# NUStatBioinfo/DegNorm

Hardware: AMD Instinct MI355X
Metric: genes/sec (20k genes x 10 samples, 5 iters) (higher is better)
Workload: dtype f64

## Files before the change

degnorm_amd/_lib.py:

```python
import ctypes
import os
import numpy as np

_HERE = os.path.dirname(os.path.abspath(__file__))
LIB_PATH = os.environ.get('DN_LIB_PATH') or os.path.join(_HERE, 'libdegnorm_amd.so')
TRACE_LEN = 48

DN_OK = 0
DN_E_INVALID, DN_E_HIP, DN_E_STATE, DN_E_UNSUPPORTED, DN_E_NO_DEVICE = -1, -2, -3, -4, -5

NMF_RANK_ONE, NMF, NMF_RATIO = 0, 1, 2
STATUS_NAMES = {0: 'ok', -1: 'ArpackError (all-zero matrix)', -2: 'empty minimum (no |K| >= 1e-5)',
                -3: 'ValueError (fewer than 2 rows or columns)', -4: 'ArpackNoConvergence (solver step cap)'}

EXIT_NAMES = ('low_cov', 'zero_sample', 'median', 'no_loop', 'refined', 'refine_fallback', 'not_found_fallback')

_lib = None


class DegnormAmdError(RuntimeError):
    pass


class Params(ctypes.Structure):
# ... 46 lines not shown
    lib.dn_debug_peek.argtypes = [vp, i32, vp]
    lib.dn_last_kernel_ms.argtypes = [vp]
    lib.dn_last_kernel_ms.restype = dbl
    lib.dn_main_kernel_name.argtypes = [vp]
    lib.dn_main_kernel_name.restype = c.c_char_p
    lib.dn_last_span_ms.argtypes = [vp]
    lib.dn_last_span_ms.restype = dbl
    lib.dn_last_init_ms.argtypes = [vp]
    lib.dn_last_init_ms.restype = dbl
    lib.dn_init_kernel_name.argtypes = [vp]
    lib.dn_init_kernel_name.restype = c.c_char_p
    lib.dn_split_length.argtypes = [vp]
    lib.dn_split_length.restype = i32
    lib.dn_class_lengths.argtypes = [vp, i32, i32, P(i32), P(i32)]
    lib.dn_class_tier_cols.argtypes = [vp, c.c_int, P(i32), P(i32)]
    lib.dn_tiny_length.argtypes = [vp]
    lib.dn_tiny_length.restype = i32
    lib.dn_class_kernel_ms.argtypes = [vp, c.c_int]
    lib.dn_class_kernel_ms.restype = dbl
    lib.dn_class_kernel_name.argtypes = [vp, c.c_int]
    lib.dn_class_kernel_name.restype = c.c_char_p
    lib.dn_synchronize.argtypes = [vp]
    lib.dn_measure_copy_gbps.argtypes = [vp, i64, c.c_int]
    lib.dn_measure_copy_gbps.restype = dbl
    lib.dn_last_rowmax_ms.argtypes = [vp]
    lib.dn_last_rowmax_ms.restype = dbl
    lib.dn_measure_read_gbps.argtypes = [vp, i64, c.c_int]
    lib.dn_measure_read_gbps.restype = dbl
    lib.dn_assemble_coverage.argtypes = [c.c_int, i64, i32, P(i64), P(vp), P(vp), i64, P(i64), i64, P(i32), P(i64), P(i64), P(i32),
                                         P(c.c_float), P(dbl)]
# ... 445 lines not shown
        return int(self.lib.dn_split_length(self.h))

    def class_lengths(self, p, downsample_rate=1):
        a, b = ctypes.c_int32(0), ctypes.c_int32(0)
        _check(self.lib.dn_class_lengths(self.h, int(p), int(downsample_rate), ctypes.byref(a), ctypes.byref(b)))
        return int(a.value), int(b.value)

    def class_tier_cols(self, cls):
        a, b = ctypes.c_int32(0), ctypes.c_int32(0)
        _check(self.lib.dn_class_tier_cols(self.h, int(cls), ctypes.byref(a), ctypes.byref(b)))
        return int(a.value), int(b.value)

    def tiny_length(self):
        return int(self.lib.dn_tiny_length(self.h))

    def class_kernel_ms(self, cls):
        return float(self.lib.dn_class_kernel_ms(self.h, int(cls)))

    def class_kernel_name(self, cls):
        return self.lib.dn_class_kernel_name(self.h, int(cls)).decode()

    def measure_copy_gbps(self, nbytes=1 << 30, reps=5):
        return float(self.lib.dn_measure_copy_gbps(self.h, int(nbytes), int(reps)))

    def measure_read_gbps(self, nbytes=1 << 30, reps=5):
        return float(self.lib.dn_measure_read_gbps(self.h, int(nbytes), int(reps)))

    def last_rowmax_ms(self):
        return float(self.lib.dn_last_rowmax_ms(self.h))
```

degnorm_amd/csrc/dn_api.hip:

```cpp
#include "dn_kernels.hpp"
#include "dn_host.hpp"
#include "../../include/degnorm_amd.h"

#include <dlfcn.h>
#include <rccl/rccl.h>

#include <algorithm>
#include <atomic>
#include <cmath>
#include <cstdio>
#include <cstdlib>
#include <cstring>
#include <memory>
#include <numeric>
#include <string>
#include <thread>
#include <vector>

#ifndef DN_P_MAX_TEMPLATED
#define DN_P_MAX_TEMPLATED 64
#endif
#define DN_P_2_16(X)  X(2) X(3) X(4) X(5) X(6) X(7) X(8) X(9) X(10) X(11) X(12) X(13) X(14) X(15) X(16)
#define DN_P_17_24(X) X(17) X(18) X(19) X(20) X(21) X(22) X(23) X(24)
#define DN_P_25_32(X) X(25) X(26) X(27) X(28) X(29) X(30) X(31) X(32)
// ... 419 lines not shown

static thread_local std::string g_err;

int dn::fail(int code, const std::string &msg) { g_err = msg; return code; }
int dn::fail_hip(const char *what, hipError_t e) { return fail(DN_E_HIP, std::string(what) + ": " + hipGetErrorString(e)); }
void dn::clear_error() { g_err.clear(); }
const char *dn::last_error() { return g_err.c_str(); }
using dn::fail;

struct dn_handle_s {
    int device = -1;
    int n_cus = 0;
    static constexpr int NCLS = 3;
    dn::Stream stream[NCLS];
    dn::Event ev_start[NCLS], ev_end[NCLS];
    dn::Event ev_ready, ev_i0, ev_i1;
    const dn::KernelSet *ks = nullptr;

    int64_t n = 0;
    int32_t p = 0;
    int64_t total = 0;
    int32_t lmax = 0;
    std::vector<int64_t> goff;
    std::vector<int32_t> glen;
    std::vector<int64_t> svoff;

    struct GeneClass {
        const dn::KernelSet *ks = nullptr;
        int32_t n = 0;
        int32_t longest = 0;
        dn::DeviceBuffer<int32_t> d_order;
        std::vector<int32_t> order;
        dn::DeviceBuffer<int32_t> d_counter;
        dn::DeviceBuffer<char> d_ws;
        int slots = 0;
        int32_t S = 0;
        int64_t slot_bytes = 0;
        int32_t lds_cols = 0;
        size_t dyn_lds = 0;
        float last_ms = 0.f;
    };
    struct DataSet {
        dn::DeviceBuffer<float> d_cov;
        dn::DeviceBuffer<int64_t> d_goff;
        dn::DeviceBuffer<int32_t> d_glen;
        dn::DeviceBuffer<int32_t> d_order;
        dn::DeviceBuffer<int32_t> d_counter;
        dn::DeviceBuffer<int64_t> d_ds;
        dn::DeviceBuffer<double> d_rho;
        dn::DeviceBuffer<int32_t> d_flags;
        dn::DeviceBuffer<int32_t> d_trace;
        dn::DeviceBuffer<double> d_kfin;
        dn::DeviceBuffer<int32_t> d_emode;
        dn::DeviceBuffer<double> d_svec;
        dn::DeviceBuffer<int64_t> d_svoff;
        dn::DeviceBuffer<float> d_rowmax;
        dn::DeviceBuffer<int32_t> d_x16;
        dn::DeviceBuffer<double> d_rhoc, d_xw, d_xadj, d_part, d_pvec;
        dn::DeviceBuffer<double> d_scales;
        dn::DeviceBuffer<double> d_x;
        dn::DeviceBuffer<uint8_t> d_ran;
        int32_t n_iter = 0;
        dn::DeviceBuffer<double> d_est_sums, d_cov_sums;
        dn::DeviceBuffer<int32_t> d_status;
        dn::DeviceBuffer<double> d_est;
        dn::DeviceBuffer<int32_t> d_tile_gene, d_tile_col;
        GeneClass cls[NCLS];
        bool have_estimate_state = false;
        dn::PinnedBuffer<int32_t> host_trace;
        size_t host_trace_len = 0;
        dn::DeviceBuffer<int32_t> d_trace_head;
// ... 163 lines not shown
    return n;
}

int dn_p_supported(int p) { return p <= dn::P_MAX && dn::kernel_set_for(p) != nullptr; }
int dn_p_max(void) { return dn::P_WIDE_MAX; }

static int create_streams(dn_handle h)
{
    int prio_least = 0, prio_greatest = 0;
    DN_TRY(hipDeviceGetStreamPriorityRange(&prio_least, &prio_greatest));
    const int prio[dn_handle_s::NCLS] = {prio_greatest, (prio_least + prio_greatest) / 2, prio_least};
    for (int c = 0; c < dn_handle_s::NCLS; c++) {
        DN_TRY(h->stream[c].create(hipStreamCreateWithPriority, hipStreamNonBlocking, prio[c]));
        DN_TRY(h->ev_start[c].create(hipEventCreate));
        DN_TRY(h->ev_end[c].create(hipEventCreate));
    }
    DN_TRY(h->ev_ready.create(hipEventCreateWithFlags, hipEventDisableTiming));
    DN_TRY(h->ev_i0.create(hipEventCreate));
    DN_TRY(h->ev_i1.create(hipEventCreate));
    return DN_OK;
}

int dn_create(int device, dn_handle *out)
{
    if (!out) return fail(DN_E_INVALID, "dn_create: out is null");
    *out = nullptr;
    int ndev = 0;
    if (hipGetDeviceCount(&ndev) != hipSuccess || ndev <= 0) return fail(DN_E_NO_DEVICE, "no HIP device visible");
    if (device < 0 || device >= ndev) return fail(DN_E_INVALID, "dn_create: device index out of range");
    DN_TRY(hipSetDevice(device));
// ... 210 lines not shown
        for (int32_t g : order) {
            const int32_t L = h->glen[g];
            ord[(h->split_len > 0 && L <= h->split_len) ? ((pair && L <= h->tiny_len) ? 2 : 1) : 0].push_back(g);
        }
        h->data.cls[0].ks = h->ks;
        h->data.cls[1].ks = (h->ks->p != 0 && h->split_len > 0) ? dn::kernel_set_narrow(p) : nullptr;
        h->data.cls[2].ks = pair;
        if (ord[0].size() >= 8) {
            const size_t n0 = ord[0].size();
            std::vector<int32_t> mixed;
            mixed.reserve(n0);
            for (size_t i = 0, j = n0 - 1; i < j; i++, j--) { mixed.push_back(ord[0][i]); mixed.push_back(ord[0][j]); }
            if (n0 & 1) mixed.push_back(ord[0][n0 / 2]);
            ord[0] = mixed;
        }
        for (int c = 0; c < dn_handle_s::NCLS; c++) {
            auto &C = h->data.cls[c];
            C.n = (int32_t) ord[c].size();
            if (C.n == 0 || !C.ks) { C.n = 0; continue; }
            DN_TRY(C.d_order.alloc(sizeof(int32_t) * (size_t) C.n));
            DN_TRY(C.d_counter.alloc(sizeof(int32_t) * 4));
            DN_TRY(hipMemcpy(C.d_order, ord[c].data(), sizeof(int32_t) * (size_t) C.n, hipMemcpyHostToDevice));
            C.order = ord[c];
            int32_t cols = C.longest = h->glen[ord[c][0]];
            if (C.ks == dn::kernel_set_rows()) cols = (cols + h->ds_hint - 1) / h->ds_hint;
            const int rc = size_class(h, C, cols);
            if (rc != DN_OK) return rc;
        }
        if (h->data.cls[0].n == 0 && (h->data.cls[1].n > 0 || h->data.cls[2].n > 0) && h->ks->p == 0) return fail(DN_E_STATE, "internal: empty wide class for the generic kernels");
        return DN_OK;
    });
    if (rc != DN_OK) {
        const std::string msg = g_err;
        free_device(h);
        h->n = 0; h->total = 0;
        return fail(rc, msg);
    }
    return DN_OK;
}

static int check_shape(dn_handle h, int64_t n_genes, int32_t p, const int64_t *lengths)
{
// ... 112 lines not shown
}

int dn_baseline_iteration(dn_handle h, const double *scale, const dn_params *prm, const int64_t *ds_start,
                          double *rho, int32_t *flags, int32_t *trace)
{
    if (!h || !h->data.d_cov) return fail(DN_E_STATE, "dn_baseline_iteration: nothing uploaded");
    if (!scale || !prm) return fail(DN_E_INVALID, "dn_baseline_iteration: null argument");
    if ((rho == nullptr) != (flags == nullptr)) return fail(DN_E_INVALID, "dn_baseline_iteration: rho and flags are fetched together or not at all");
    { const int rc = check_params(prm, ds_start, h->n, [&](int64_t g) { return h->glen[g]; }); if (rc != DN_OK) return rc; }
    for (int i = 0; i < h->p; i++) if (!(scale[i] > 0.0) || !std::isfinite(scale[i])) return fail(DN_E_INVALID, "scale factors must be positive and finite");
    DN_TRY(hipSetDevice(h->device));
    return synced_classes(h, [&]() -> int {
        const int32_t rate = prm->downsample_rate;
        for (auto &C : h->data.cls) {
            if (C.n == 0 || !C.ks) continue;
            const int32_t longest = C.longest;
            const int32_t need = rate > 1 ? (longest + rate - 1) / rate : longest;
            if (need > C.S) {
                DN_TRY(hipStreamSynchronize(h->stream[0]));
                const int rc = size_class(h, C, need);
                if (rc != DN_OK) return rc;
            }
        }
        if (prm->want_estimates && !h->data.d_svec)
            DN_TRY(h->data.d_svec.alloc(sizeof(double) * (size_t) std::max<int64_t>(h->svoff[h->n], 1)));

        dn::IterArgs a;
        std::memset(&a, 0, sizeof(a));
        a.cov = h->data.d_cov; a.goff = h->data.d_goff; a.glen = h->data.d_glen; a.order = h->data.d_order; a.counter = h->data.d_counter;
        a.ds_start = nullptr;
        a.ws = h->data.cls[0].d_ws; a.rho = h->data.d_rho; a.flags = h->data.d_flags; a.trace = h->data.d_trace; a.kfin = h->data.d_kfin; a.emode = h->data.d_emode;
// ... 19 lines not shown
            const double per_call = 4.0 * (double) (C.ks->nt > 0 ? C.ks->nt : 128);
            std::vector<std::pair<double, int32_t>> key((size_t) C.n);
            for (int32_t k = 0; k < C.n; k++) {
                const int32_t g = C.order[k];
                const int32_t *tr = &h->data.host_trace[(size_t) g * h->trace_cols];
                key[k] = {(double) tr[2] + per_call * (double) tr[1] + 1e-3 * (double) h->glen[g], g};
            }
            std::stable_sort(key.begin(), key.end(), [](const std::pair<double, int32_t> &a, const std::pair<double, int32_t> &b) { return a.first > b.first; });
            for (int32_t k = 0; k < C.n; k++) C.order[k] = key[k].second;
            DN_TRY(hipMemcpyAsync(C.d_order, C.order.data(), sizeof(int32_t) * (size_t) C.n, hipMemcpyHostToDevice, h->stream[0]));
        }
        DN_TRY(hipMemsetAsync(h->data.d_trace, 0, sizeof(int32_t) * (size_t) h->n * dn::TRACE_LEN, h->stream[0]));
        for (auto &C : h->data.cls) if (C.n > 0) DN_TRY(hipMemsetAsync(C.d_counter, 0, sizeof(int32_t) * 4, h->stream[0]));
        DN_TRY(hipEventRecord(h->ev_ready, h->stream[0]));
        int first_cls = -1;
        for (int c = 0; c < dn_handle_s::NCLS; c++) {
            auto &C = h->data.cls[c];
            C.last_ms = 0.f;
            if (C.n == 0) continue;
            if (first_cls < 0) first_cls = c;
            hipStream_t st = h->stream[c];
            if (c > 0) DN_TRY(hipStreamWaitEvent(st, h->ev_ready, 0));
            a.order = C.d_order; a.counter = C.d_counter; a.ws = C.d_ws; a.slot_bytes = C.slot_bytes; a.S = C.S;
            a.lds_cols = C.lds_cols; a.n_genes = C.n;
            DN_TRY(hipEventRecord(h->ev_start[c], st));
            const int lrc = C.ks->baseline_ptr ? C.ks->baseline_ptr(a, h->data.d_scales, C.slots, st) : C.ks->baseline(a, C.slots, C.dyn_lds, st);
            if (lrc != 0) return fail(DN_E_HIP, std::string("k_baseline launch: ") + hipGetErrorString((hipError_t) lrc));
            DN_TRY(hipEventRecord(h->ev_end[c], st));
        }
        for (int c = 1; c < dn_handle_s::NCLS; c++)
            if (h->data.cls[c].n > 0) DN_TRY(hipStreamWaitEvent(h->stream[0], h->ev_end[c], 0));
        if (rho) {
            DN_TRY(hipMemcpyAsync(rho, h->data.d_rho, sizeof(double) * (size_t) h->n * h->p, hipMemcpyDeviceToHost, h->stream[0]));
            DN_TRY(hipMemcpyAsync(flags, h->data.d_flags, sizeof(int32_t) * (size_t) h->n, hipMemcpyDeviceToHost, h->stream[0]));
        }
        const int32_t tcols = h->trace_cols;
        const size_t trace_ints = (size_t) h->n * (size_t) tcols;
        if (h->data.host_trace_len < trace_ints) {
            h->data.host_trace_len = 0;
            DN_TRY(h->data.host_trace.alloc(sizeof(int32_t) * trace_ints));
            h->data.host_trace_len = trace_ints;
        }
        if (tcols == dn::TRACE_LEN)
            DN_TRY(hipMemcpyAsync(h->data.host_trace, h->data.d_trace, sizeof(int32_t) * trace_ints, hipMemcpyDeviceToHost, h->stream[0]));
        else {
            if (!h->data.d_trace_head) DN_TRY(h->data.d_trace_head.alloc(sizeof(int32_t) * (size_t) h->n * dn::TRACE_LEN));
            hipLaunchKernelGGL(k_trace_head, dim3((unsigned) std::min<size_t>(1024, (trace_ints + 255) / 256)), dim3(256), 0, h->stream[0],
                               h->data.d_trace, h->data.d_trace_head, (long long) trace_ints, (int) tcols);
            DN_TRY(hipGetLastError());
            DN_TRY(hipMemcpyAsync(h->data.host_trace, h->data.d_trace_head, sizeof(int32_t) * trace_ints, hipMemcpyDeviceToHost, h->stream[0]));
        }
        DN_TRY(hipStreamSynchronize(h->stream[0]));
        h->have_trace = (prm->downsample_rate <= 1);
        if (trace) std::memcpy(trace, h->data.host_trace, sizeof(int32_t) * trace_ints);
        h->last_span_ms = 0.f;
        for (int c = 0; c < dn_handle_s::NCLS; c++) {
            if (h->data.cls[c].n == 0) continue;
            DN_TRY(hipEventElapsedTime(&h->data.cls[c].last_ms, h->ev_start[c], h->ev_end[c]));
            float span = 0.f;
            DN_TRY(hipEventElapsedTime(&span, h->ev_start[first_cls], h->ev_end[c]));
            h->last_span_ms = std::max(h->last_span_ms, span);
        }
        h->last_ms = first_cls >= 0 ? h->data.cls[first_cls].last_ms : 0.f;
        h->data.have_estimate_state = prm->want_estimates != 0;
        return DN_OK;
    });
}
// ... 565 lines not shown
        return DN_OK;
    });
}

double dn_last_f64_ms(dn_handle h) { return h ? (double) h->last_f64_ms : 0.0; }

double dn_last_kernel_ms(dn_handle h) { return h ? (double) h->last_ms : 0.0; }
double dn_last_init_ms(dn_handle h) { return h ? (double) h->last_init_ms : 0.0; }
double dn_last_span_ms(dn_handle h) { return h ? (double) h->last_span_ms : 0.0; }
double dn_last_rowmax_ms(dn_handle h) { return h ? (double) h->last_rowmax_ms : 0.0; }
const char *dn_init_kernel_name(dn_handle h) { return h ? h->init_name : ""; }
const char *dn_main_kernel_name(dn_handle h) { return (h && h->ks) ? h->ks->baseline_name : ""; }
double dn_class_kernel_ms(dn_handle h, int cls) { return (h && cls >= 0 && cls < dn_handle_s::NCLS) ? (double) h->data.cls[cls].last_ms : 0.0; }
const char *dn_class_kernel_name(dn_handle h, int cls) { return (h && cls >= 0 && cls < dn_handle_s::NCLS && h->data.cls[cls].ks && h->data.cls[cls].n > 0) ? h->data.cls[cls].ks->baseline_name : ""; }
int32_t dn_tiny_length(dn_handle h) { return h ? h->tiny_len : 0; }
int dn_class_tier_cols(dn_handle h, int cls, int32_t *reg_cols, int32_t *lds_cols)
{
    if (!h || cls < 0 || cls >= dn_handle_s::NCLS || !reg_cols || !lds_cols) return fail(DN_E_INVALID, "dn_class_tier_cols: bad argument");
    const auto &C = h->data.cls[cls];
    const bool live = C.ks && C.n > 0;
    *reg_cols = live ? C.ks->reg_tier_cols : 0;
    *lds_cols = live ? C.lds_cols : 0;
    return DN_OK;
}
int dn_class_lengths(dn_handle h, int32_t p, int32_t downsample_rate, int32_t *split_len, int32_t *tiny_len)
{
    if (!h || !split_len || !tiny_len) return fail(DN_E_INVALID, "dn_class_lengths: null argument");
    const dn::KernelSet *ks = dn::kernel_set_for(p);
    if (!ks) return fail(DN_E_UNSUPPORTED, "no kernels compiled for p = " + std::to_string(p));
    DN_TRY(hipSetDevice(h->device));
// ... 104 lines not shown
```

degnorm_amd/csrc/dn_kernels.hpp:

```cpp
#pragma once
#include <hip/hip_runtime.h>
#include <stddef.h>
#include <stdint.h>
#include <type_traits>
#include "dn_reduce.hpp"
#include "dn_dpp_ops.hpp"

#ifdef DN_MARKS
#define DN_MARK(name) asm volatile("; DN_MARK " name)
#else
#define DN_MARK(name)
#endif

namespace dn {

constexpr int TRACE_LEN = 48;
constexpr int MAX_BINS = 64;
constexpr int P_MAX = 64;
constexpr int P_WIDE_MAX = 256;

enum { EXIT_LOW_COV = 0, EXIT_ZERO_SAMPLE = 1, EXIT_MEDIAN = 2, EXIT_NO_LOOP = 3,
       EXIT_REFINED = 4, EXIT_REFINE_FALLBACK = 5, EXIT_NOT_FOUND_FALLBACK = 6 };
enum { LOOP_NATURAL = 0, LOOP_PERFECT = 1, LOOP_VALUE_ERROR = 2, LOOP_ZERO_ROWSUM = 3, LOOP_MIN_BINS = 4,
       LOOP_NOT_ENTERED = 5 };
// ... 19 lines not shown
    char          *ws;
    double        *rho;
    int32_t       *flags;
    int32_t       *trace;
    double        *kfin;
    int32_t       *emode;
    double        *svec;
    const int64_t *svoff;
    int64_t        slot_bytes;
    int32_t        n_genes;
    int32_t        S;
    int32_t        lds_cols;
    int32_t        T, bins, min_hc, rate, skip, want_est;
    int32_t        p;
    int32_t        max_steps;
};

struct IterArgs : IterFields<float> { double scale[P_MAX], inv_scale[P_MAX]; };

struct IterArgsF64 : IterFields<double> { double scale[P_MAX], inv_scale[P_MAX]; };

struct WideIterArgs : IterFields<float> { const double *scale, *inv_scale; };

struct InitArgs {
    const float   *cov;
    const int64_t *goff;
    const int32_t *glen;
    const int32_t *order;
    int32_t       *counter;
    double        *est_sums;
    double        *cov_sums;
// ... 18 lines not shown
    const double  *svec;
    const int64_t *svoff;
    double        *out;
    const int64_t *ooff;
    int32_t        n_genes;
    int32_t        p;
};
struct EstArgs : EstFields<float> { double scale[P_MAX]; };
struct EstArgsF64 : EstFields<double> { double scale[P_MAX]; };
struct WideEstArgs : EstFields<float> { const double *scale; };

#pragma clang diagnostic push
#pragma clang diagnostic ignored "-Winvalid-offsetof"
template <typename A> constexpr bool iter_layout_kept()
{
    return sizeof(A) == 1208 && offsetof(A, slot_bytes) == 128 && offsetof(A, p) == 172 && offsetof(A, scale) == 184 &&
           offsetof(A, inv_scale) == 696;
}
template <typename A> constexpr bool est_layout_kept() { return sizeof(A) == 592 && offsetof(A, p) == 76 && offsetof(A, scale) == 80; }
static_assert(iter_layout_kept<IterArgs>() && iter_layout_kept<IterArgsF64>(), "IterArgs / IterArgsF64: layout moved");
static_assert(est_layout_kept<EstArgs>() && est_layout_kept<EstArgsF64>(), "EstArgs / EstArgsF64: layout moved");
#pragma clang diagnostic pop

struct NmfArgsF64 {
    const double  *x;
    const int64_t *xoff;
    const int32_t *ncol;
    const int64_t *eoff;
    const int32_t *order;
    int32_t       *counter;
    double        *K;
    double        *E;
// ... 1650 lines not shown
    if (DN_TIDX == 0) g_gs.stamp[3] += __builtin_amdgcn_s_memtime() - t_call0;
#endif
}


template <int P> __device__ __forceinline__ double lds_max(const double *v)
{ double m = v[0];
#pragma unroll
  for (int i = 1; i < P; i++) { const double t = v[i]; m = t > m ? t : m; } return m; }
template <int P> __device__ __forceinline__ double lds_min(const double *v)
{ double m = v[0];
#pragma unroll
  for (int i = 1; i < P; i++) { const double t = v[i]; m = t < m ? t : m; } return m; }

template <int P, int NT>
__global__ __launch_bounds__(NT * DN_UNITS, DN_KERNEL_WAVES) void k_baseline(IterArgs A)
{
    constexpr int W = NT / 64;
    Smem<P, NT> &sm = g_sm;
    GeneState<P> &gs = g_gs;
    const int tid = DN_TIDX, lane = lane_id(), w = wave_id();
    const int S = A.S;
    const int nL = A.lds_cols;
    char *slot = A.ws + ((size_t) blockIdx.x * DN_UNITS + DN_UNIT) * A.slot_bytes;
    float *Fs = reinterpret_cast<float *>(slot);
    float *Fb = Fs + (size_t) P * S;
    double *Lg = reinterpret_cast<double *>(Fb + (size_t) P * S);
    double *sv = Lg + (size_t) (P + (P & 1)) * S;
    double *rs = sv + S;
    double *rtsave = rs + 2 * (size_t) S;
// ... 9 lines not shown
            diag = diag || (t == i * (i + 1) / 2 + i);
            if (t >= i * (i + 1) / 2) { ra = i; rb = t - i * (i + 1) / 2; }
        }
        if constexpr (P <= 16) sm.sqi[t] = (t < P * (P + 1) / 2) ? (ra * Smem<P, NT>::SQ_STR + rb) | ((rb * Smem<P, NT>::SQ_STR + ra) << 16) : 0;
        if constexpr (raw_units<P>())
            sm.dsel[t] = (t < P * (P + 1) / 2) ? (diag ? -1.0 : 1.0) * A.inv_scale[ra] * A.inv_scale[rb < P ? rb : 0] : 0.0;
        else sm.dsel[t] = diag ? 1.0 : 0.0;
        if (t == Smem<P, NT>::ZSLOT) sm.tot[t] = 0.0;
    }

    for (;;) {
        if (tid == 0) sm.gene = atomicAdd(A.counter, 1);
        dn_sync();
        const int q = sm.gene;
        dn_sync();
        if (q >= A.n_genes) break;
        const int g = A.order[q];
        const int L = A.glen[g];
        const float *x = A.cov + A.goff[g];

        int n0 = 0, n_calls = 0, n_drops = 0, exit_code = EXIT_LOW_COV, loop_reason = LOOP_NOT_ENTERED;
        int status = ST_OK, flag = 0, emode = EM_INPUT;
        long long sum_cols = 0;
#ifdef DN_STAMP
        const long long t_gene0 = __builtin_amdgcn_s_memtime();
        long long t_ret = 0, t_book = 0;
#endif
        int32_t *tr = A.trace + (size_t) g * TRACE_LEN;
        if (tid < P) { gs.rho[tid] = 0.0; gs.K[tid] = 0.0; gs.us[tid] = 0.0; }
        if (tid == 0) { gs.steps = 0; gs.stamp[0] = gs.stamp[1] = gs.stamp[2] = gs.stamp[3] = gs.stamp[4] = gs.stamp[5] = 0; }
#ifdef DN_STAMP
        if (tid == 0) gs.stamp[6] = gs.stamp[7] = 0;
#endif

        double thr;
        int x16;
        {
            const float *rmx = A.rowmax + (size_t) g * P;
            double gmax = (double) rmx[0] / A.scale[0];
#pragma unroll
            for (int i = 1; i < P; i++) { const double v = (double) rmx[i] / A.scale[i]; gmax = v > gmax ? v : gmax; }
// ... 51 lines not shown
            if (n0 >= A.min_hc) {
                block_sum<P, P, NT>(sumF, sm);
                if (tid == 0) {
#pragma unroll
                    for (int i = 0; i < P; i++) gs.sumF[i] = sumF[i];
                }
            }
            dn_sync();
        }

#ifdef DN_STAMP
        const long long t_scan1 = __builtin_amdgcn_s_memtime();
#endif
        int n = n0;
        if (n0 >= A.min_hc) {
            if (!(lds_min<P>(gs.sumF) > 0.0)) exit_code = EXIT_ZERO_SAMPLE;
            else {
                const double min_gene_len = fmax(2.0, ceil(200.0 * (1.0 / (double) rate)));
                const double min_bins = ceil((double) A.bins * 0.2);
                int csize = 1, n_bins = 0;
                bool first = true, in_loop = false;
                for (;;) {
#ifdef DN_STAMP
                    if (t_ret != 0) t_book += __builtin_amdgcn_s_memtime() - t_ret;
#endif
                    nmf_call<P, NT>(Fb, Lg, rs, sv, rtsave, n, S, nL, A.T, first ? 1 : 0, x16);
                    if constexpr (P < DN_MG_MIN_P) {
                        const int st_call = __builtin_amdgcn_readfirstlane(gs.status);
                        bool unsafe = st_call == ST_NO_CONVERGENCE;
                        if (st_call == ST_OK) {
#pragma unroll
                            for (int i = 0; i < P; i++)
                                unsafe = unsafe || (gs.u[i] < WARM_START_MIN_COMPONENT && gs.sums[1 + P + i] > 0.0);
                        }
                        if (__builtin_amdgcn_readfirstlane((int) unsafe) != 0) {
                            dn_sync();
                            nmf_call<P, NT, true>(Fb, Lg, rs, sv, rtsave, n, S, nL, A.T, first ? 1 : 0, x16);
                        }
                    }
#ifdef DN_STAMP
                    t_ret = __builtin_amdgcn_s_memtime();
#endif
                    if (gs.status != ST_OK) { status = gs.status; break; }
                    const double *u = gs.u, *sums = gs.sums;
                    const double theta = gs.theta;
                    n_calls++; sum_cols += n;
                    if (first) {
                        if (tid == 0) {
                            const double sig = sqrt(theta);
                            gs.sig0 = sig;
#pragma unroll
                            for (int i = 0; i < P; i++) {
                                gs.us[i] = u[i];
                                gs.K[i] = u[i] * sig;
                                gs.rho[i] = 1.0 - sums[1 + P + i] / (u[i] * sums[0] + 1.0);
                                gs.rho_fb[i] = 1.0 - gs.sumF[i] / (sums[1 + i] + 1.0);
// ... 52 lines not shown
                    dn_sync();
                    double best = -INFINITY; int drop = 0;
                    for (int b = 0; b < n_bins; b++) { const double v = sm.ss[b]; if (v > best) { best = v; drop = b; } }
                    dn_sync();
                    if (best == 0.0) { loop_reason = LOOP_PERFECT; break; }
                    const int kb = drop * csize;
                    const int dlen = ((kb + csize < n) ? kb + csize : n) - kb;
                    if (tid == 0) {
                        for (int b = drop; b < n_bins - 1; b++) sm.alive[b] = sm.alive[b + 1];
                        if (n_drops < 32) tr[8 + n_drops] = drop;
                    }
                    n_bins--;
                    n -= dlen;
                    n_drops++;
                    dn_sync();
                    for (int k0 = kb + tid; k0 < n; k0 += 4 * NT) {
                        float v[4][P];
#pragma unroll
                        for (int c = 0; c < 4; c++) {
                            const int k = (k0 + c * NT < n) ? k0 + c * NT : k0;
                            const int a = k / csize;
                            const int ko = sm.alive[a] * csize + (k - a * csize);
#pragma unroll
                            for (int i = 0; i < P; i++) v[c][i] = Fs[(size_t) i * S + ko];
                        }
#pragma unroll
                        for (int c = 0; c < 4; c++) {
                            if (k0 + c * NT < n) {
#pragma unroll
                                for (int i = 0; i < P; i++) Fb[(size_t) (k0 + c * NT) * P + i] = v[c][i];
                            }
                        }
                    }
                    dn_sync();
                    if (n < 2) { loop_reason = LOOP_VALUE_ERROR; break; }
                }

                if (in_loop && status == ST_OK) {
                    bool fallback = false;
                    if (lds_max<P>(gs.rho) < 0.2) {
                        double K[P];
#pragma unroll
                        for (int i = 0; i < P; i++) K[i] = gs.K[i];
                        status = fix_k<P>(K);
                        if (status == ST_OK) {
                            double se[1] = {0.0};
                            for (int k = tid; k < n0; k += NT) {
                                double m = -INFINITY;
#pragma unroll
                                for (int i = 0; i < P; i++) {
                                    const double qv = ((double) Fs[(size_t) i * S + k] * gs.inv[i]) / K[i];
                                    m = qv > m ? qv : m;
                                }
// ... 14 lines not shown
#pragma unroll
                                    for (int i = 0; i < P; i++) { gs.K[i] = K[i]; gs.rho[i] = 1.0 - gs.sumF[i] / (K[i] * se[0] + 1.0); }
                                }
                            }
                        }
                    } else { fallback = true; exit_code = EXIT_NOT_FOUND_FALLBACK; }
                    if (fallback && status == ST_OK) {
                        if (tid == 0) {
#pragma unroll
                            for (int i = 0; i < P; i++) { gs.K[i] = gs.us[i] * gs.sig0; gs.rho[i] = gs.rho_fb[i]; }
                        }
                        emode = (n0 < L) ? EM_EXPAND : EM_CLAMPED;
                    }
                    dn_sync();
                }
                if (status == ST_OK && exit_code >= EXIT_NO_LOOP && n0 < L) {
                    double K[P];
#pragma unroll
                    for (int i = 0; i < P; i++) K[i] = gs.K[i];
                    status = fix_k<P>(K);
                    dn_sync();
                    if (tid == 0) {
#pragma unroll
                        for (int i = 0; i < P; i++) gs.K[i] = K[i];
                    }
                }
            }
        }
        dn_sync();

        const bool zero_out = (status != ST_OK) || exit_code <= EXIT_MEDIAN;
        if (zero_out) { emode = EM_INPUT; if (status != ST_OK) flag = 0; }

        if (tid == 0) {
#pragma unroll
            for (int i = 0; i < P; i++) {
                A.rho[(size_t) g * P + i] = zero_out ? 0.0 : gs.rho[i];
                A.kfin[(size_t) g * P + i] = (emode == EM_CLAMPED || emode == EM_RAW) ? gs.us[i] : gs.K[i];
            }
            A.flags[g] = flag;
            A.emode[g] = emode;
            tr[0] = n0; tr[1] = n_calls; tr[2] = (int32_t) sum_cols; tr[3] = exit_code; tr[4] = loop_reason;
            tr[5] = n_drops; tr[6] = status; tr[7] = gs.steps;
#ifdef DN_STAMP
            tr[40] = (int32_t) (gs.stamp[0] >> 10); tr[41] = (int32_t) (gs.stamp[1] >> 10); tr[42] = (int32_t) (gs.stamp[2] >> 10);
            tr[44] = (int32_t) (gs.stamp[3] >> 10); tr[45] = (int32_t) (gs.stamp[4] >> 10); tr[46] = (int32_t) (gs.stamp[5] >> 10);
            tr[43] = (int32_t) ((__builtin_amdgcn_s_memtime() - t_gene0) >> 10);
            tr[47] = (int32_t) ((t_scan1 - t_gene0) >> 10);
            tr[39] = (int32_t) (t_book >> 10);
            tr[38] = (int32_t) ((t_ret != 0 ? __builtin_amdgcn_s_memtime() - t_ret : 0) >> 10);
            tr[36] = (int32_t) (gs.stamp[6] >> 10); tr[37] = (int32_t) gs.stamp[7];
#endif
        }
        if (A.want_est && (emode == EM_CLAMPED || emode == EM_RAW)) {
            double *dst = A.svec + A.svoff[g];
            for (int k = tid; k < n0; k += NT) dst[k] = sv[k];
        }
        dn_sync();
    }
}

template <int P, int NT>
__global__ __launch_bounds__(NT) void k_ratio_svd(InitArgs A)
{
    constexpr int NG = P * (P + 1) / 2;
    Smem<P, NT> &sm = g_sm;
    const int tid = DN_TIDX;
    for (;;) {
        if (tid == 0) sm.gene = atomicAdd(A.counter, 1);
// ... 135 lines not shown
```

include/degnorm_amd.h:

```cpp
#ifndef DEGNORM_AMD_H
#define DEGNORM_AMD_H

#include <stdint.h>

#ifdef __cplusplus
extern "C" {
#endif

#define DN_OK                 0
#define DN_E_INVALID         -1
#define DN_E_HIP             -2
#define DN_E_STATE           -3
#define DN_E_UNSUPPORTED     -4
#define DN_E_NO_DEVICE       -5

#define DN_TRACE_LEN          48

typedef struct dn_handle_s *dn_handle;

typedef struct {
    int32_t nmf_iter;
    int32_t bins;
    int32_t min_high_coverage;
    int32_t downsample_rate;
// ... 249 lines not shown
                       int64_t *gene_beg, int32_t *gene_len, uint64_t *gene_hash, int64_t *n_nodes, int64_t *n_walked, int64_t *err_line,
                       int32_t *err_kind);

double dn_last_kernel_ms(dn_handle h);
const char *dn_main_kernel_name(dn_handle h);
double dn_last_init_ms(dn_handle h);
double dn_last_rowmax_ms(dn_handle h);
const char *dn_init_kernel_name(dn_handle h);
int32_t dn_split_length(dn_handle h);
int  dn_class_lengths(dn_handle h, int32_t p, int32_t downsample_rate, int32_t *split_len, int32_t *tiny_len);
int32_t dn_tiny_length(dn_handle h);
double dn_class_kernel_ms(dn_handle h, int cls);
double dn_last_span_ms(dn_handle h);
const char *dn_class_kernel_name(dn_handle h, int cls);
int  dn_class_tier_cols(dn_handle h, int cls, int32_t *reg_cols, int32_t *lds_cols);
int  dn_synchronize(dn_handle h);
double dn_measure_copy_gbps(dn_handle h, int64_t bytes, int reps);
double dn_measure_read_gbps(dn_handle h, int64_t bytes, int reps);

#ifdef __cplusplus
}
#endif
#endif
```

Baseline: 15600.

## Hand down shrunken genes from wider size class to narrower class kernel

While a gene in a wider size class iterates, once its remaining column count drops below what the next narrower class can hold, the block saves its loop state (counters, rho, K, alive bins) to global memory and parks the gene on the next class's queue. After the donor kernel finishes, the next class's stream waits on an event and launches a continuation kernel that restores the state, rebuilds the working matrix and finishes the loop with the smaller-footprint kernel. The aim is to stop large-footprint, low-occupancy blocks from spending their tail iterations on data that now fits the cheaper kernel. The cost is extra global state traffic, an added kernel launch and a cross-stream dependency that serialises the continuation behind the whole donor kernel. The path is disabled when estimates are requested, when downsampling is used, or when bins exceed a fixed cap.

```diff
diff --git a/degnorm_amd/_lib.py b/degnorm_amd/_lib.py
--- a/degnorm_amd/_lib.py
+++ b/degnorm_amd/_lib.py
@@ -84,6 +84,9 @@
     lib.dn_split_length.restype = i32
     lib.dn_class_lengths.argtypes = [vp, i32, i32, P(i32), P(i32)]
     lib.dn_class_tier_cols.argtypes = [vp, c.c_int, P(i32), P(i32)]
+    if hasattr(lib, 'dn_handdown'):
+        lib.dn_handdown.argtypes = [vp, c.c_int, P(i32), P(i32)]
+        lib.dn_handdown.restype = c.c_int
     lib.dn_tiny_length.argtypes = [vp]
     lib.dn_tiny_length.restype = i32
     lib.dn_class_kernel_ms.argtypes = [vp, c.c_int]
@@ -559,6 +562,11 @@
     def tiny_length(self):
         return int(self.lib.dn_tiny_length(self.h))
 
+    def handdown(self, cls):
+        a, b = ctypes.c_int32(0), ctypes.c_int32(0)
+        _check(self.lib.dn_handdown(self.h, int(cls), ctypes.byref(a), ctypes.byref(b)))
+        return int(a.value), int(b.value)
+
     def class_kernel_ms(self, cls):
         return float(self.lib.dn_class_kernel_ms(self.h, int(cls)))
 
diff --git a/degnorm_amd/csrc/dn_api.hip b/degnorm_amd/csrc/dn_api.hip
--- a/degnorm_amd/csrc/dn_api.hip
+++ b/degnorm_amd/csrc/dn_api.hip
@@ -457,6 +457,7 @@
     static constexpr int NCLS = 3;
     dn::Stream stream[NCLS];
     dn::Event ev_start[NCLS], ev_end[NCLS];
+    dn::Event ev_mid[NCLS];
     dn::Event ev_ready, ev_i0, ev_i1;
     const dn::KernelSet *ks = nullptr;
 
@@ -472,6 +473,10 @@
         const dn::KernelSet *ks = nullptr;
         int32_t n = 0;
         int32_t longest = 0;
+        int32_t recv_longest = 0;
+        int32_t hand_cols = 0;
+        dn::DeviceBuffer<int32_t> d_inq;
+        int32_t parked = 0;
         dn::DeviceBuffer<int32_t> d_order;
         std::vector<int32_t> order;
         dn::DeviceBuffer<int32_t> d_counter;
@@ -498,6 +503,9 @@
         dn::DeviceBuffer<double> d_svec;
         dn::DeviceBuffer<int64_t> d_svoff;
         dn::DeviceBuffer<float> d_rowmax;
+        dn::PinnedBuffer<int32_t> host_parked;
+        dn::DeviceBuffer<int32_t> d_hand_int;
+        dn::DeviceBuffer<double> d_hand_dbl;
         dn::DeviceBuffer<int32_t> d_x16;
         dn::DeviceBuffer<double> d_rhoc, d_xw, d_xadj, d_part, d_pvec;
         dn::DeviceBuffer<double> d_scales;
@@ -691,6 +699,7 @@
         DN_TRY(h->stream[c].create(hipStreamCreateWithPriority, hipStreamNonBlocking, prio[c]));
         DN_TRY(h->ev_start[c].create(hipEventCreate));
         DN_TRY(h->ev_end[c].create(hipEventCreate));
+        DN_TRY(h->ev_mid[c].create(hipEventCreateWithFlags, hipEventDisableTiming));
     }
     DN_TRY(h->ev_ready.create(hipEventCreateWithFlags, hipEventDisableTiming));
     DN_TRY(h->ev_i0.create(hipEventCreate));
@@ -931,6 +940,8 @@
             if (n0 & 1) mixed.push_back(ord[0][n0 / 2]);
             ord[0] = mixed;
         }
+        const char *henv = getenv("DN_HANDDOWN");
+        const bool handdown = h->ks->p != 0 && !h->ks->baseline_ptr && !(henv && henv[0] == '0');
         for (int c = 0; c < dn_handle_s::NCLS; c++) {
             auto &C = h->data.cls[c];
             C.n = (int32_t) ord[c].size();
@@ -940,9 +951,31 @@
             DN_TRY(hipMemcpy(C.d_order, ord[c].data(), sizeof(int32_t) * (size_t) C.n, hipMemcpyHostToDevice));
             C.order = ord[c];
             int32_t cols = C.longest = h->glen[ord[c][0]];
+            C.recv_longest = 0; C.hand_cols = 0; C.parked = 0;
+            if (handdown && c > 0 && h->data.cls[c - 1].n > 0) {
+                C.recv_longest = h->data.cls[c - 1].longest;
+                DN_TRY(C.d_inq.alloc(sizeof(int32_t) * (size_t) h->data.cls[c - 1].n));
+                cols = std::max(cols, C.recv_longest);
+            }
             if (C.ks == dn::kernel_set_rows()) cols = (cols + h->ds_hint - 1) / h->ds_hint;
             const int rc = size_class(h, C, cols);
             if (rc != DN_OK) return rc;
+        }
+        {
+            int32_t over[2] = {-1, -1};
+            if (const char *cenv = getenv("DN_HANDDOWN_COLS")) (void) sscanf(cenv, "%d,%d", &over[0], &over[1]);
+            bool any = false;
+            for (int c = 0; c + 1 < dn_handle_s::NCLS; c++) {
+                const auto &R = h->data.cls[c + 1];
+                if (h->data.cls[c].n == 0 || R.n == 0 || h->ks->p == 0 || h->ks->baseline_ptr) continue;
+                h->data.cls[c].hand_cols = over[c] >= 0 ? over[c] : R.ks->reg_tier_cols + R.lds_cols;
+                any = any || (R.recv_longest > 0 && h->data.cls[c].hand_cols > 0);
+            }
+            if (any) {
+                DN_TRY(h->data.host_parked.alloc(sizeof(int32_t) * dn_handle_s::NCLS));
+                DN_TRY(h->data.d_hand_int.alloc(sizeof(int32_t) * (size_t) n * dn::HAND_INTS));
+                DN_TRY(h->data.d_hand_dbl.alloc(sizeof(double) * (size_t) n * (size_t) (5 * p + 1)));
+            }
         }
         if (h->data.cls[0].n == 0 && (h->data.cls[1].n > 0 || h->data.cls[2].n > 0) && h->ks->p == 0) return fail(DN_E_STATE, "internal: empty wide class for the generic kernels");
         return DN_OK;
@@ -1085,7 +1118,7 @@
         const int32_t rate = prm->downsample_rate;
         for (auto &C : h->data.cls) {
             if (C.n == 0 || !C.ks) continue;
-            const int32_t longest = C.longest;
+            const int32_t longest = std::max(C.longest, C.recv_longest);
             const int32_t need = rate > 1 ? (longest + rate - 1) / rate : longest;
             if (need > C.S) {
                 DN_TRY(hipStreamSynchronize(h->stream[0]));
@@ -1135,6 +1168,8 @@
         for (auto &C : h->data.cls) if (C.n > 0) DN_TRY(hipMemsetAsync(C.d_counter, 0, sizeof(int32_t) * 4, h->stream[0]));
         DN_TRY(hipEventRecord(h->ev_ready, h->stream[0]));
         int first_cls = -1;
+        const bool hand_ok = h->data.d_hand_int && !prm->want_estimates && prm->downsample_rate <= 1 && prm->bins <= dn::HAND_MAX_BINS;
+        bool donor_parks = false, parked_from[dn_handle_s::NCLS] = {false, false, false};
         for (int c = 0; c < dn_handle_s::NCLS; c++) {
             auto &C = h->data.cls[c];
             C.last_ms = 0.f;
@@ -1144,13 +1179,31 @@
             if (c > 0) DN_TRY(hipStreamWaitEvent(st, h->ev_ready, 0));
             a.order = C.d_order; a.counter = C.d_counter; a.ws = C.d_ws; a.slot_bytes = C.slot_bytes; a.S = C.S;
             a.lds_cols = C.lds_cols; a.n_genes = C.n;
+            C.parked = 0;
+            a.handdown_cols = C.hand_cols;
+            a.hand_int = h->data.d_hand_int; a.hand_dbl = h->data.d_hand_dbl;
+            a.park_queue = nullptr; a.park_count = nullptr; a.resume_queue = nullptr; a.resume_count = nullptr;
+            const bool parks = hand_ok && c + 1 < dn_handle_s::NCLS && C.hand_cols > 0 && h->data.cls[c + 1].recv_longest > 0 && h->data.cls[c + 1].n > 0;
+            if (parks) { a.park_queue = h->data.cls[c + 1].d_inq; a.park_count = h->data.cls[c + 1].d_counter + 2; }
             DN_TRY(hipEventRecord(h->ev_start[c], st));
             const int lrc = C.ks->baseline_ptr ? C.ks->baseline_ptr(a, h->data.d_scales, C.slots, st) : C.ks->baseline(a, C.slots, C.dyn_lds, st);
             if (lrc != 0) return fail(DN_E_HIP, std::string("k_baseline launch: ") + hipGetErrorString((hipError_t) lrc));
+            if (parks) DN_TRY(hipEventRecord(h->ev_mid[c], st));
+            if (c > 0 && donor_parks) {
+                DN_TRY(hipStreamWaitEvent(st, h->ev_mid[c - 1], 0));
+                a.park_queue = nullptr; a.park_count = nullptr;
+                a.counter = C.d_counter + 1; a.resume_queue = C.d_inq; a.resume_count = C.d_counter + 2;
+                const int lrc2 = C.ks->baseline(a, C.slots, C.dyn_lds, st);
+                if (lrc2 != 0) return fail(DN_E_HIP, std::string("k_baseline launch (continuations): ") + hipGetErrorString((hipError_t) lrc2));
+            }
             DN_TRY(hipEventRecord(h->ev_end[c], st));
+            parked_from[c] = c > 0 && donor_parks;
+            donor_parks = parks;
         }
         for (int c = 1; c < dn_handle_s::NCLS; c++)
             if (h->data.cls[c].n > 0) DN_TRY(hipStreamWaitEvent(h->stream[0], h->ev_end[c], 0));
+        for (int c = 1; c < dn_handle_s::NCLS; c++)
+            if (parked_from[c]) DN_TRY(hipMemcpyAsync(h->data.host_parked + (c - 1), h->data.cls[c].d_counter + 2, sizeof(int32_t), hipMemcpyDeviceToHost, h->stream[0]));
         if (rho) {
             DN_TRY(hipMemcpyAsync(rho, h->data.d_rho, sizeof(double) * (size_t) h->n * h->p, hipMemcpyDeviceToHost, h->stream[0]));
             DN_TRY(hipMemcpyAsync(flags, h->data.d_flags, sizeof(int32_t) * (size_t) h->n, hipMemcpyDeviceToHost, h->stream[0]));
@@ -1172,6 +1225,7 @@
             DN_TRY(hipMemcpyAsync(h->data.host_trace, h->data.d_trace_head, sizeof(int32_t) * trace_ints, hipMemcpyDeviceToHost, h->stream[0]));
         }
         DN_TRY(hipStreamSynchronize(h->stream[0]));
+        for (int c = 1; c < dn_handle_s::NCLS; c++) if (parked_from[c]) h->data.cls[c - 1].parked = h->data.host_parked[c - 1];
         h->have_trace = (prm->downsample_rate <= 1);
         if (trace) std::memcpy(trace, h->data.host_trace, sizeof(int32_t) * trace_ints);
         h->last_span_ms = 0.f;
@@ -1767,6 +1821,15 @@
 double dn_class_kernel_ms(dn_handle h, int cls) { return (h && cls >= 0 && cls < dn_handle_s::NCLS) ? (double) h->data.cls[cls].last_ms : 0.0; }
 const char *dn_class_kernel_name(dn_handle h, int cls) { return (h && cls >= 0 && cls < dn_handle_s::NCLS && h->data.cls[cls].ks && h->data.cls[cls].n > 0) ? h->data.cls[cls].ks->baseline_name : ""; }
 int32_t dn_tiny_length(dn_handle h) { return h ? h->tiny_len : 0; }
+
+int dn_handdown(dn_handle h, int cls, int32_t *cols, int32_t *parked)
+{
+    if (!h || !cols || !parked) return fail(DN_E_INVALID, "dn_handdown: null argument");
+    if (cls < 0 || cls >= dn_handle_s::NCLS) return fail(DN_E_INVALID, "dn_handdown: no such class");
+    *cols = h->data.cls[cls].hand_cols;
+    *parked = h->data.cls[cls].parked;
+    return DN_OK;
+}
 int dn_class_tier_cols(dn_handle h, int cls, int32_t *reg_cols, int32_t *lds_cols)
 {
     if (!h || cls < 0 || cls >= dn_handle_s::NCLS || !reg_cols || !lds_cols) return fail(DN_E_INVALID, "dn_class_tier_cols: bad argument");
diff --git a/degnorm_amd/csrc/dn_kernels.hpp b/degnorm_amd/csrc/dn_kernels.hpp
--- a/degnorm_amd/csrc/dn_kernels.hpp
+++ b/degnorm_amd/csrc/dn_kernels.hpp
@@ -57,7 +57,16 @@
     int32_t        T, bins, min_hc, rate, skip, want_est;
     int32_t        p;
     int32_t        max_steps;
+    int32_t        handdown_cols;
+    int32_t       *hand_int;
+    double        *hand_dbl;
+    int32_t       *park_queue;
+    int32_t       *park_count;
+    const int32_t *resume_queue;
+    const int32_t *resume_count;
 };
+constexpr int HAND_MAX_BINS = 32;
+constexpr int HAND_INTS = 16 + HAND_MAX_BINS;
 
 struct IterArgs : IterFields<float> { double scale[P_MAX], inv_scale[P_MAX]; };
 
@@ -106,8 +115,8 @@
 #pragma clang diagnostic ignored "-Winvalid-offsetof"
 template <typename A> constexpr bool iter_layout_kept()
 {
-    return sizeof(A) == 1208 && offsetof(A, slot_bytes) == 128 && offsetof(A, p) == 172 && offsetof(A, scale) == 184 &&
-           offsetof(A, inv_scale) == 696;
+    return sizeof(A) == 1256 && offsetof(A, slot_bytes) == 128 && offsetof(A, p) == 172 && offsetof(A, hand_int) == 184 &&
+           offsetof(A, scale) == 232 && offsetof(A, inv_scale) == 744;
 }
 template <typename A> constexpr bool est_layout_kept() { return sizeof(A) == 592 && offsetof(A, p) == 76 && offsetof(A, scale) == 80; }
 static_assert(iter_layout_kept<IterArgs>() && iter_layout_kept<IterArgsF64>(), "IterArgs / IterArgsF64: layout moved");
@@ -1788,6 +1797,29 @@
   for (int i = 1; i < P; i++) { const double t = v[i]; m = t < m ? t : m; } return m; }
 
 template <int P, int NT>
+__device__ __forceinline__ void rebuild_fb(const float *Fs, float *Fb, const int32_t *alive, int S, int csize, int n, int kb, int tid)
+{
+    for (int k0 = kb + tid; k0 < n; k0 += 4 * NT) {
+        float v[4][P];
+#pragma unroll
+        for (int c = 0; c < 4; c++) {
+            const int k = (k0 + c * NT < n) ? k0 + c * NT : k0;
+            const int a = k / csize;
+            const int ko = alive[a] * csize + (k - a * csize);
+#pragma unroll
+            for (int i = 0; i < P; i++) v[c][i] = Fs[(size_t) i * S + ko];
+        }
+#pragma unroll
+        for (int c = 0; c < 4; c++) {
+            if (k0 + c * NT < n) {
+#pragma unroll
+                for (int i = 0; i < P; i++) Fb[(size_t) (k0 + c * NT) * P + i] = v[c][i];
+            }
+        }
+    }
+}
+
+template <int P, int NT>
 __global__ __launch_bounds__(NT * DN_UNITS, DN_KERNEL_WAVES) void k_baseline(IterArgs A)
 {
     constexpr int W = NT / 64;
@@ -1827,17 +1859,20 @@
         dn_sync();
         const int q = sm.gene;
         dn_sync();
-        if (q >= A.n_genes) break;
-        const int g = A.order[q];
+        const bool resume = A.resume_queue != nullptr;
+        if (q >= (resume ? *A.resume_count : A.n_genes)) break;
+        const int g = resume ? A.resume_queue[q] : A.order[q];
         const int L = A.glen[g];
         const float *x = A.cov + A.goff[g];
+        bool parked = false;
 
         int n0 = 0, n_calls = 0, n_drops = 0, exit_code = EXIT_LOW_COV, loop_reason = LOOP_NOT_ENTERED;
         int status = ST_OK, flag = 0, emode = EM_INPUT;
         long long sum_cols = 0;
 #ifdef DN_STAMP
         const long long t_gene0 = __builtin_amdgcn_s_memtime();
-        long long t_ret = 0, t_book = 0;
+        long long t_ret = 0, t_book = 0, t_hand = 0;
+        int n_hand = 0;
 #endif
         int32_t *tr = A.trace + (size_t) g * TRACE_LEN;
         if (tid < P) { gs.rho[tid] = 0.0; gs.K[tid] = 0.0; gs.us[tid] = 0.0; }
@@ -1919,15 +1954,55 @@
 #endif
         int n = n0;
         if (n0 >= A.min_hc) {
-            if (!(lds_min<P>(gs.sumF) > 0.0)) exit_code = EXIT_ZERO_SAMPLE;
+            if (!resume && !(lds_min<P>(gs.sumF) > 0.0)) exit_code = EXIT_ZERO_SAMPLE;
             else {
                 const double min_gene_len = fmax(2.0, ceil(200.0 * (1.0 / (double) rate)));
                 const double min_bins = ceil((double) A.bins * 0.2);
                 int csize = 1, n_bins = 0;
                 bool first = true, in_loop = false;
+                if (resume) {
+                    const int32_t *ri = A.hand_int + (size_t) g * HAND_INTS;
+                    const double *rd = A.hand_dbl + (size_t) g * (5 * P + 1);
+                    n = ri[1]; csize = ri[2]; n_bins = ri[3]; n_calls = ri[4]; n_drops = ri[5];
+                    sum_cols = (long long) (((unsigned long long) (uint32_t) ri[7] << 32) | (unsigned long long) (uint32_t) ri[6]);
+                    flag = ri[8]; exit_code = ri[9]; loop_reason = ri[10]; emode = ri[11];
+                    if (tid < n_bins) sm.alive[tid] = ri[16 + tid];
+                    if (tid == 0) {
+                        gs.steps = ri[12];
+#pragma unroll
+                        for (int i = 0; i < P; i++) {
+                            gs.rho[i] = rd[i]; gs.K[i] = rd[P + i]; gs.us[i] = rd[2 * P + i]; gs.rho_fb[i] = rd[3 * P + i]; gs.sumF[i] = rd[4 * P + i];
+                        }
+                        gs.sig0 = rd[5 * P];
+                    }
+                    first = false; in_loop = true;
+                    dn_sync();
+                    rebuild_fb<P, NT>(Fs, Fb, sm.alive, S, csize, n, 0, tid);
+                    dn_sync();
+                }
                 for (;;) {
+                    if (A.park_queue != nullptr && !first && in_loop && n <= A.handdown_cols) {
+                        int32_t *ri = A.hand_int + (size_t) g * HAND_INTS;
+                        double *rd = A.hand_dbl + (size_t) g * (5 * P + 1);
+                        if (tid < n_bins) ri[16 + tid] = sm.alive[tid];
+                        if (tid == 0) {
+                            ri[0] = n0; ri[1] = n; ri[2] = csize; ri[3] = n_bins; ri[4] = n_calls; ri[5] = n_drops;
+                            ri[6] = (int32_t) (uint32_t) (unsigned long long) sum_cols; ri[7] = (int32_t) (uint32_t) ((unsigned long long) sum_cols >> 32);
+                            ri[8] = flag; ri[9] = exit_code; ri[10] = loop_reason; ri[11] = emode; ri[12] = gs.steps;
+#pragma unroll
+                            for (int i = 0; i < P; i++) {
+                                rd[i] = gs.rho[i]; rd[P + i] = gs.K[i]; rd[2 * P + i] = gs.us[i]; rd[3 * P + i] = gs.rho_fb[i]; rd[4 * P + i] = gs.sumF[i];
+                            }
+                            rd[5 * P] = gs.sig0;
+                            A.park_queue[atomicAdd(A.park_count, 1)] = g;
+                        }
+                        parked = true;
+                        break;
+                    }
 #ifdef DN_STAMP
                     if (t_ret != 0) t_book += __builtin_amdgcn_s_memtime() - t_ret;
+                    const long long t_call = __builtin_amdgcn_s_memtime();
+                    const bool hand = !first && in_loop && n <= A.handdown_cols;
 #endif
                     nmf_call<P, NT>(Fb, Lg, rs, sv, rtsave, n, S, nL, A.T, first ? 1 : 0, x16);
                     if constexpr (P < DN_MG_MIN_P) {
@@ -1945,6 +2020,7 @@
                     }
 #ifdef DN_STAMP
                     t_ret = __builtin_amdgcn_s_memtime();
+                    if (hand) { t_hand += t_ret - t_call; n_hand++; }
 #endif
                     if (gs.status != ST_OK) { status = gs.status; break; }
                     const double *u = gs.u, *sums = gs.sums;
@@ -2027,29 +2103,12 @@
                     n -= dlen;
                     n_drops++;
                     dn_sync();
-                    for (int k0 = kb + tid; k0 < n; k0 += 4 * NT) {
-                        float v[4][P];
-#pragma unroll
-                        for (int c = 0; c < 4; c++) {
-                            const int k = (k0 + c * NT < n) ? k0 + c * NT : k0;
-                            const int a = k / csize;
-                            const int ko = sm.alive[a] * csize + (k - a * csize);
-#pragma unroll
-                            for (int i = 0; i < P; i++) v[c][i] = Fs[(size_t) i * S + ko];
-                        }
-#pragma unroll
-                        for (int c = 0; c < 4; c++) {
-                            if (k0 + c * NT < n) {
-#pragma unroll
-                                for (int i = 0; i < P; i++) Fb[(size_t) (k0 + c * NT) * P + i] = v[c][i];
-                            }
-                        }
-                    }
+                    rebuild_fb<P, NT>(Fs, Fb, sm.alive, S, csize, n, kb, tid);
                     dn_sync();
                     if (n < 2) { loop_reason = LOOP_VALUE_ERROR; break; }
                 }
 
-                if (in_loop && status == ST_OK) {
+                if (in_loop && status == ST_OK && !parked) {
                     bool fallback = false;
                     if (lds_max<P>(gs.rho) < 0.2) {
                         double K[P];
@@ -2094,7 +2153,7 @@
                     }
                     dn_sync();
                 }
-                if (status == ST_OK && exit_code >= EXIT_NO_LOOP && n0 < L) {
+                if (status == ST_OK && exit_code >= EXIT_NO_LOOP && n0 < L && !parked) {
                     double K[P];
 #pragma unroll
                     for (int i = 0; i < P; i++) K[i] = gs.K[i];
@@ -2112,7 +2171,7 @@
         const bool zero_out = (status != ST_OK) || exit_code <= EXIT_MEDIAN;
         if (zero_out) { emode = EM_INPUT; if (status != ST_OK) flag = 0; }
 
-        if (tid == 0) {
+        if (tid == 0 && !parked) {
 #pragma unroll
             for (int i = 0; i < P; i++) {
                 A.rho[(size_t) g * P + i] = zero_out ? 0.0 : gs.rho[i];
@@ -2129,10 +2188,11 @@
             tr[47] = (int32_t) ((t_scan1 - t_gene0) >> 10);
             tr[39] = (int32_t) (t_book >> 10);
             tr[38] = (int32_t) ((t_ret != 0 ? __builtin_amdgcn_s_memtime() - t_ret : 0) >> 10);
+            tr[35] = (int32_t) (t_hand >> 10); tr[34] = n_hand;
             tr[36] = (int32_t) (gs.stamp[6] >> 10); tr[37] = (int32_t) gs.stamp[7];
 #endif
         }
-        if (A.want_est && (emode == EM_CLAMPED || emode == EM_RAW)) {
+        if (A.want_est && !parked && (emode == EM_CLAMPED || emode == EM_RAW)) {
             double *dst = A.svec + A.svoff[g];
             for (int k = tid; k < n0; k += NT) dst[k] = sv[k];
         }
diff --git a/include/degnorm_amd.h b/include/degnorm_amd.h
--- a/include/degnorm_amd.h
+++ b/include/degnorm_amd.h
@@ -287,6 +287,7 @@
 double dn_last_span_ms(dn_handle h);
 const char *dn_class_kernel_name(dn_handle h, int cls);
 int  dn_class_tier_cols(dn_handle h, int cls, int32_t *reg_cols, int32_t *lds_cols);
+int  dn_handdown(dn_handle h, int cls, int32_t *cols, int32_t *parked);
 int  dn_synchronize(dn_handle h);
 double dn_measure_copy_gbps(dn_handle h, int64_t bytes, int reps);
 double dn_measure_read_gbps(dn_handle h, int64_t bytes, int reps);
```

After: 16040 (median of 6 runs). 1.03x the previous value.
